# PSeitz/veloci

Measured on AMD Instinct MI355X. Metric: queries/sec, 3-term AND on 100M-doc index (p50 latency and HBM fraction alongside), higher is better.
Workload: dtype u32 doc ids + f16->f32 scores

## Files before the change

veloci_amd/csrc/capi.cpp:

```cpp
#include <chrono>
#include <thread>
#include <cstdio>
#include <cstdlib>
#include <cstring>

#include "../../include/veloci_amd.h"
#include <functional>
#include <future>

#include <dlfcn.h>
#include <unistd.h>

#include "engine.hpp"
#include "text.hpp"

using namespace vq;
using vqreq::Request;
using vqreq::VelociError;

namespace {
thread_local std::string g_err;

int fail(int code, const std::string& msg) {
    g_err = msg;
// ... 1440 lines not shown
        c->nccl = comm;
        comm_setup(idx, std::move(c));
        idx.allreduce_fn = comm_sum_u64;
        idx.allreduce_ctx = &idx;
    });
}
int vq_comm_init_custom(vq_index* index, int nranks, int rank, vq_allgather_fn allgather, vq_allreduce_u32_fn allreduce_u32, void* ctx) {
    return guard([&] {
        if (!index || !allgather || nranks < 1 || rank < 0 || rank >= nranks) throw VelociError(VQ_ERR_INVALID_ARGUMENT, "vq_comm_init_custom: bad argument");
        auto c = std::make_unique<ShardComm>();
        c->nranks = nranks;
        c->rank = rank;
        c->allgather = allgather;
        c->allreduce_u32 = allreduce_u32;
        c->ctx = ctx;
        comm_release(*index->idx, "vq_comm_init_custom");
        comm_setup(*index->idx, std::move(c));
    });
}
int vq_comm_destroy(vq_index* index) {
    return guard([&] {
        if (!index) throw VelociError(VQ_ERR_INVALID_ARGUMENT, "vq_comm_destroy: null index");
        comm_release(*index->idx, "vq_comm_destroy");
    });
}

struct vq_shard_step {
    const Index* idx = nullptr;
    std::vector<std::unique_ptr<PartialBatch>> pbs;
    std::vector<size_t> first, arena_off;
    size_t n = 0, used = 0;
    int parity = 0;
    bool merge_queued = false;
    bool counted = false;
    ~vq_shard_step() {
        pbs.clear();
        if (idx && idx->comm && idx->comm->unmerged == this) idx->comm->unmerged = nullptr;
        if (counted && idx && idx->comm) {
            idx->comm->live -= 1;
            idx->comm->busy[parity] = false;
        }
    }
};
namespace {
void comm_fail(ShardComm& c, const std::string& why) {
    if (!c.failed.empty()) return;
    c.failed = why;
    if (c.nccl) {
        try {
            if (rccl_api().CommAbort) (void)rccl_api().CommAbort(static_cast<ncclComm_t>(c.nccl));
            c.nccl = nullptr;
        } catch (...) {
        }
    }
}
void bounded_wait(const Index& idx, ShardComm& c, hipEvent_t ev) {
    static const long limit_ms = [] {
        const char* e = std::getenv("VQ_STEP_TIMEOUT_MS");
        return e ? std::atol(e) : 120000L;
    }();
    const auto t0 = std::chrono::steady_clock::now();
    for (uint64_t spins = 0;; ++spins) {
        const hipError_t q = hipEventQuery(ev);
        if (q == hipSuccess) return;
        if (q != hipErrorNotReady) {
            comm_fail(c, std::string("the step's stream reported ") + hipGetErrorString(q));
            throw VelociError(VQ_ERR_DEVICE, "sharded step: " + c.failed);
        }
        if (spins < 2000) continue;
        if ((spins & 63u) == 0) {
            if (c.nccl && rccl_api().CommGetAsyncError) {
                int aerr = 0;
                if (rccl_api().CommGetAsyncError(static_cast<ncclComm_t>(c.nccl), &aerr) == 0 && aerr != 0) {
                    comm_fail(c, std::string("RCCL reported ") + (rccl_api().GetErrorString ? rccl_api().GetErrorString(aerr) : "an error") + " while the step was in flight (a rank is gone)");
                    throw VelociError(VQ_ERR_DEVICE, "sharded step: " + c.failed);
                }
            }
            const long waited = long(std::chrono::duration_cast<std::chrono::milliseconds>(std::chrono::steady_clock::now() - t0).count());
            if (limit_ms > 0 && waited > limit_ms) {
                comm_fail(c, "a step did not complete within " + std::to_string(limit_ms) + " ms (VQ_STEP_TIMEOUT_MS): a rank did not join its exchange");
                throw VelociError(VQ_ERR_DEVICE, "sharded step: " + c.failed);
            }
        }
        std::this_thread::sleep_for(std::chrono::microseconds(20));
    }
    (void)idx;
}
void step_queue_merge(vq_shard_step& step) {
    if (step.merge_queued) return;
    step.merge_queued = true;
    const Index& idx = *step.idx;
    ShardComm& c = *idx.comm;
    if (c.unmerged == &step) c.unmerged = nullptr;
    if (step.used) VQ_HIP(hipStreamWaitEvent(idx.fin_stream, c.ev_xchg[step.parity], 0));
    const uint8_t* gathered = static_cast<const uint8_t*>(c.gathered[step.parity].p);
    for (size_t k = 0; k < step.pbs.size(); ++k)
        finish_launch(idx, *step.pbs[k], step.used && step.pbs[k]->nq_dev ? gathered + step.arena_off[k] : nullptr, uint32_t(c.nranks));
    VQ_HIP(hipEventRecord(c.ev_fin[step.parity], idx.fin_stream));
}
}

int vq_shard_step_begin(const vq_index* index, const vq_request* const* requests, size_t n, vq_shard_step** out) {
    return guard([&] {
        if (!index || !out || (n && !requests)) throw VelociError(VQ_ERR_INVALID_ARGUMENT, "vq_shard_step_begin: null argument");
        *out = nullptr;
        const Index& idx = *index->idx;
        if (!idx.comm) {
            auto local = std::make_unique<ShardComm>();
            comm_setup(const_cast<Index&>(idx), std::move(local));
        }
        ShardComm& c = *idx.comm;
        if (!c.failed.empty()) throw VelociError(VQ_ERR_DEVICE, "vq_shard_step_begin: the communicator is down (" + c.failed + "): make it again (vq_comm_init / vq_comm_init_custom) on every rank");
        const bool exchange = c.nccl != nullptr || c.allgather != nullptr;
        static const bool timing = std::getenv("VQ_TIMING") != nullptr;
        const auto tb0 = std::chrono::steady_clock::now();
        VQ_HIP(hipSetDevice(idx.device));
        const std::vector<const Request*> reqs = request_pointers(requests, n);
        if (c.unmerged) {
            vq_shard_step& prev = *static_cast<vq_shard_step*>(c.unmerged);
            step_queue_merge(prev);
            VQ_HIP(hipStreamWaitEvent(idx.stream, c.ev_fin[prev.parity], 0));
        }
        const auto tb1 = std::chrono::steady_clock::now();
        if (c.live >= 2) throw VelociError(VQ_ERR_INVALID_ARGUMENT, "vq_shard_step_begin: two steps are in flight already (end one first)");
        auto step = std::make_unique<vq_shard_step>();
        step->idx = &idx;
        step->counted = true;
        c.live += 1;
        step->n = n;
        step->parity = c.busy[0] ? 1 : 0;
        if (c.busy[step->parity]) {
            step->counted = false;
            c.live -= 1;
            throw VelociError(VQ_ERR_INVALID_ARGUMENT, "vq_shard_step_begin: both step slots are held (end a step first)");
        }
        c.busy[step->parity] = true;
        auto tb2 = tb1;
        try {
        const size_t chunks_env = [] {
            const char* e = std::getenv("VQ_SHARD_CHUNKS");
            return size_t(e ? std::min(2, std::max(1, std::atoi(e))) : 0);
        }();
        const size_t nchunks = chunks_env && n >= 512 ? chunks_env : 1;
        for (size_t k = 0; k < nchunks; ++k) {
            const size_t b = n * k / nchunks, e = n * (k + 1) / nchunks;
            step->first.push_back(b);
            step->pbs.push_back(run_partial(idx, reqs.data() + b, e - b, step->parity * 2 + int(k)));
        }
        tb2 = std::chrono::steady_clock::now();
        size_t off = 0;
        for (auto& pb : step->pbs) {
            step->arena_off.push_back(off);
            if (exchange && pb->nq_dev) off += (size_t(pb->layout.off_hist) * size_t(c.nranks) + 255) / 256 * 256;
        }
// ... 132 lines not shown
```

veloci_amd/csrc/device_types.hpp:

```cpp
#pragma once
#include <hip/hip_runtime.h>
#include <stdint.h>

namespace vq {

constexpr int kBlock = 64;
constexpr int kCandCap = 2048;
constexpr int kMaxTopK = 1024;
constexpr int kStackDepth = 16;
constexpr int kMaxChildren = 16;
constexpr int kMaxLists = 64;
constexpr int kMaxOps = 160;
constexpr int kMaxSkipWhen = 4;
constexpr uint32_t kTileDirShift = 14;
constexpr uint32_t kProbeTileShift = 15;
static_assert(kProbeTileShift == 15, "an arr16 entry holds a 15-bit in-tile offset and a class bit");
constexpr uint32_t kArrPadRel = (1u << kProbeTileShift) - 1u;
#ifndef VQ_SCORE_CLASS_DIV
#define VQ_SCORE_CLASS_DIV 8
#endif
constexpr uint32_t kScoreClassDiv = VQ_SCORE_CLASS_DIV;
constexpr uint32_t kRankShift = 9;

enum ListFlags : uint32_t {
// ... 105 lines not shown
};

constexpr int kWideMax = 16;
struct DWide {
    uint8_t n_leaves, n_groups, root_kind, root_nslots;
    uint8_t seq, pad0, pad1, pad2;
    uint16_t bitmap_mask, cover_mask, prefetch_mask, f32_mask;
    uint16_t leaf_list[kWideMax];
    uint8_t leaf_slot[kWideMax];
    uint8_t g_kind[kWideMax], g_begin[kWideMax], g_count[kWideMax];
    uint8_t leaf_and_order[kWideMax];
    uint8_t leaf_slot_order[kWideMax];
    uint8_t r_and_order[kWideMax];
    uint8_t r_slot[kWideMax];
    uint8_t r_slot_order[kWideMax];
};

struct QHeader {
    uint32_t n_lists, n_ops, n_fops, n_groups, n_tboost, n_col, n_locf, n_facets;
    uint32_t off_lists, off_ops, off_fops, off_groups, off_tboost, off_col, off_locf, off_facets;
    uint32_t top_k;
    uint32_t tile_words;
    uint32_t n_spans;
    uint32_t keys_base;
    uint32_t doc_lo, doc_hi;
    uint32_t part_keys_off;
    uint32_t blob_bytes;
    uint32_t desc_bytes;
    uint32_t n_pres, off_pres, off_pres_in, n_temps;
    uint32_t off_loc_idx;
    uint32_t off_simple2;
    uint32_t off_pool;
    uint32_t prune_n;
    uint64_t prune_mask;
    unsigned long long gthr;
    unsigned long long key_upper;
    uint32_t seq_tiles;
    uint32_t stat_off;
    uint32_t prune_gbits[16];
    uint32_t n_counts;
    uint32_t bitmap_base;
    uint32_t simple_n;
    uint32_t simple_flags;
};

constexpr uint32_t kSfBitmapShift = 0;
constexpr uint32_t kSfCoverShift = 8;
constexpr uint32_t kSfArrayShift = 12;
constexpr uint32_t kSfPrefetchShift = 20;
constexpr uint32_t kSfLeafMask = 0xFu;
constexpr uint32_t kSfSeq = 1u << 16;
constexpr uint32_t kSfSimple = 1u << 17;
constexpr uint32_t kSfRich = 1u << 18;
constexpr uint32_t kSfLeafF32 = 1u << 19;
constexpr uint32_t kSfWide = 1u << 24;
constexpr uint32_t kSfProbe = 1u << 25;
constexpr uint32_t kSfProbeOr = 1u << 27;
constexpr uint32_t kSfUnionPacked = 1u << 28;
__host__ __device__ inline uint32_t sf_bitmap_mask(uint32_t f) { return (f >> kSfBitmapShift) & kSfLeafMask; }
__host__ __device__ inline uint32_t sf_cover_mask(uint32_t f) { return (f >> kSfCoverShift) & kSfLeafMask; }
__host__ __device__ inline uint32_t sf_array_mask(uint32_t f) { return (f >> kSfArrayShift) & kSfLeafMask; }
__host__ __device__ inline uint32_t sf_prefetch_mask(uint32_t f) { return (f >> kSfPrefetchShift) & kSfLeafMask; }
__host__ __device__ inline bool sf_bitmap(uint32_t f, uint32_t k) { return (f >> (kSfBitmapShift + k)) & 1u; }
__host__ __device__ inline bool sf_cover(uint32_t f, uint32_t k) { return (f >> (kSfCoverShift + k)) & 1u; }
__host__ __device__ inline bool sf_array(uint32_t f, uint32_t k) { return (f >> (kSfArrayShift + k)) & 1u; }
__host__ __device__ inline bool sf_prefetch(uint32_t f, uint32_t k) { return (f >> (kSfPrefetchShift + k)) & 1u; }
__host__ __device__ inline bool sf_seq(uint32_t f) { return (f & kSfSeq) != 0u; }
__host__ __device__ inline bool sf_rich(uint32_t f) { return (f & kSfRich) != 0u; }
__host__ __device__ inline bool sf_leaf_f32(uint32_t f) { return (f & kSfLeafF32) != 0u; }
__host__ __device__ inline bool sf_wide(uint32_t f) { return (f & kSfWide) != 0u; }
__host__ __device__ inline bool sf_probe(uint32_t f) { return (f & kSfProbe) != 0u; }
__host__ __device__ inline bool sf_probe_or(uint32_t f) { return (f & kSfProbeOr) != 0u; }
__host__ __device__ inline bool sf_union_packed(uint32_t f) { return (f & kSfUnionPacked) != 0u; }

struct DProbeLeaf {
    const uint32_t* cov32;
    const uint16_t* arr16;
// ... 21 lines not shown
```

veloci_amd/csrc/engine.hpp:

```cpp
#pragma once
#include <hip/hip_runtime.h>

#include <atomic>
#include <cmath>
#include <chrono>
#include <cstdint>
#include <cstdlib>
#include <map>
#include <limits>
#include <memory>
#include <thread>
#include <functional>
#include <condition_variable>
#include <mutex>
#include <string>
#include <unordered_map>
#include <vector>

#include "device_types.hpp"
#include "kernels.hpp"
#include "request.hpp"
#include "hostpool.hpp"
#include "regex_dfa.hpp"

// ... 373 lines not shown
struct PinnedBuf {
    void* p = nullptr;
    size_t bytes = 0;
    PinnedBuf() = default;
    PinnedBuf(const PinnedBuf&) = delete;
    PinnedBuf& operator=(const PinnedBuf&) = delete;
    ~PinnedBuf();
    void ensure(size_t n);
    template <class T>
    T* as() const { return reinterpret_cast<T*>(p); }
};

constexpr int kWorkspaces = 4;

enum KernelId : int {
    K_DICT_SCAN = 0, K_DICT_REGEX, K_DICT_TOPN_GROUP, K_DICT_TOPN, K_TEXT_BEST, K_TEXT_SELECT, K_UNION_COUNT, K_UNION_WRITE, K_UNION_DENSE_SCATTER, K_UNION_DENSE_COUNT, K_UNION_DENSE_WRITE, K_RANGE_HITS, K_COUNT_PREPASS, K_SCAN_LEAF_F32, K_SCAN_RICH, K_SCAN_PROBE, K_SCAN_AND, K_SCAN_SIMPLE, K_SCAN_UNION,
    K_SCAN_WIDE, K_TILE_SCAN, K_MERGE_SPANS, K_FINALIZE, K_FACET_SELECT, K_LOCALITY, K_BOOST1N, K_COUNT_
};
extern const char* const kKernelNames[K_COUNT_];

struct TimedLaunch {
    int kernel;
    uint32_t ev_begin, ev_end;
    uint64_t layout_bytes, algorithmic_bytes, queries;
};

struct Workspace {
    std::mutex mu;
    std::atomic<bool> pinned{false};
    std::vector<hipEvent_t> ev_pool;
    uint32_t ev_used = 0;
    std::vector<TimedLaunch> timed;
    hipEvent_t ev_done = nullptr;
    PinnedBuf h_up, h_down;
    DevBuf d_up;
    DevBuf d_span_keys;
    DevBuf d_partial;
    DevBuf d_down;
    DevBuf d_union_docs[2], d_union_vals[2], d_union_max, d_union_meta;
    DevBuf d_union_slab, d_union_dense_docs, d_union_dense_vals, d_union_dense_meta;
    DevBuf d_loc_a, d_loc_b, d_loc_pairs_a, d_loc_pairs_b, d_loc_meta, d_loc_tmp, d_loc_docs, d_loc_vals;
    DevBuf d_b1n_a, d_b1n_b, d_b1n_meta, d_b1n_tmp, d_b1n_docs, d_b1n_vals;
    DevBuf d_probe_desc, d_probe_counts, d_probe_ids;
    DevBuf d_regex_tabs;
    DevBuf d_topn_sort, d_topn_tmp, d_topn_meta, d_topn_out;
    DevBuf d_trank_best, d_trank_meta;
};

struct KernelProfile {
    double ms = 0;
    uint64_t launches = 0;
    uint64_t layout_bytes = 0;
    uint64_t algorithmic_bytes = 0;
    uint64_t gathered_bytes = 0;
    uint64_t queries = 0;
};
struct Profile {
    bool enabled = false;
    KernelProfile k[K_COUNT_];
    uint64_t batches = 0;
};
struct LaunchTimer {
    Workspace* ws = nullptr;
    hipStream_t st = nullptr;
    size_t slot = 0;
    LaunchTimer(bool on, Workspace& w, hipStream_t s, int kernel, uint64_t layout_bytes = 0, uint64_t algorithmic_bytes = 0, uint64_t queries = 0);
// ... 248 lines not shown
    bool has_facets = false;
    std::map<std::string, std::vector<std::string>> why_found_terms;
    std::shared_ptr<const ExplainPlan> explain_plan;
    std::shared_ptr<const WhyFoundPlan> why_found_plan;
    std::map<uint32_t, std::map<std::string, std::vector<std::string>>> why_found_info;
    bool has_explain = false;
    std::vector<std::pair<bool, ExplainRecs>> explain;
    bool deep = false;
    bool rerun_exact = false;
    mutable std::string json;
};

struct PartialBatch {
    const Index* index = nullptr;
    Workspace* ws = nullptr;
    std::unique_lock<std::mutex> lock;
    bool pinned_ws = false;
    std::vector<CompiledQuery> queries;
    std::vector<uint32_t> slot;
    std::vector<uint8_t> qclass;
    std::vector<FacetJob> facet_jobs;
    uint32_t nq_dev = 0;
    PartialLayout layout{};
    const uint8_t* d_blobs = nullptr;
    const uint32_t* d_blob_off = nullptr;
    const FacetJob* d_facet_jobs = nullptr;
    uint8_t* d_partial = nullptr;
    uint32_t total_spans = 0;
    uint32_t n_facet_jobs = 0;
    uint32_t total_facet_out = 0;
    bool profiled = false;
    bool launched = false, finished = false;
    bool merge_launched = false;
    std::chrono::steady_clock::time_point t0;
    void release_workspace();
    std::vector<const vqreq::Request*> reqs;
    ~PartialBatch();
};

std::unique_ptr<PartialBatch> run_partial(const Index& idx, const vqreq::Request* const* reqs, size_t n, int slot = -1, int64_t arena_offset = -1);
void finish_batch(const Index& idx, PartialBatch& pb, const void* gathered_device, uint32_t num_shards, std::vector<std::unique_ptr<Result>>& out,
                  std::vector<int>& status, std::vector<std::string>& errors, size_t shard_stride = 0);
void finish_launch(const Index& idx, PartialBatch& pb, const void* gathered_device, uint32_t num_shards, size_t shard_stride = 0);

}
```

veloci_amd/csrc/exec.cpp:

```cpp
#include <algorithm>
#include <cstdio>
#include <cstdlib>
#include <cstring>
#include <thread>

#include "engine.hpp"
#include "staging.hpp"

#include "text.hpp"

namespace vq {

using namespace vqreq;

void DevBuf::ensure(size_t n) {
    if (n <= bytes) return;
    size_t want = std::max(n, bytes + bytes / 2);
    alloc(want);
}
PinnedBuf::~PinnedBuf() {
    if (p) (void)hipHostFree(p);
}
void PinnedBuf::ensure(size_t n) {
    if (n <= bytes) return;
// ... 641 lines not shown
                P.facets_rich = P.facets_rich || !cq.facets.empty();
                P.scatter_rich = std::max<uint32_t>(P.scatter_rich, n_scatter + cq.simple2.n_side);
                break;
            case K_SCAN_UNION: P.union_has_or = P.union_has_or || cq.simple_n > 1; break;
            case K_SCAN_PROBE: {
                ScanPlan::ProbeParams& pp = P.probe[ti - T_PROBE];
                pp.na_seen |= 1u << uint32_t(__builtin_popcount(sf_array_mask(cq.simple_flags)));
                pp.arr_slot = std::max(pp.arr_slot, cq.probe_arr_gran * 4u);
                P.any_probe = true;
                break;
            }
            case K_SCAN_AND: P.scatter_and = std::max(P.scatter_and, n_scatter); break;
            case K_SCAN_SIMPLE: P.scatter_simple = std::max(P.scatter_simple, n_scatter); break;
            default: break;
        }
        pb.qclass.push_back(uint8_t(cq.kclass));
        P.cls_layout[cq.kclass] += cq.layout_bytes;
        P.cls_algo[cq.kclass] += cq.algorithmic_bytes;
        P.cls_q[cq.kclass] += 1;
        ++qi;
    }
    for (ScanTable& t : P.tabs) t.span_base[t.n] = t.spans;
    if (!pb.facet_jobs.empty()) std::memcpy(hup + up_jobs, pb.facet_jobs.data(), pb.facet_jobs.size() * sizeof(FacetJob));
    pb.d_blobs = dup;
    pb.d_blob_off = reinterpret_cast<const uint32_t*>(dup + up_blob_off);
    pb.d_facet_jobs = reinterpret_cast<const FacetJob*>(dup + up_jobs);
    return P;
}

static void launch_scans(const Index& idx, PartialBatch& pb, const BatchLayout& L, const ScanPlan& P, int64_t arena_offset) {
    Workspace& ws = *pb.ws;
    const PartialLayout& lay = pb.layout;
    hipStream_t st = idx.stream;
    VQ_HIP(hipMemcpyAsync(ws.d_up.as<uint8_t>(), ws.h_up.as<uint8_t>(), P.up_bytes, hipMemcpyHostToDevice, st));
    ws.d_span_keys.ensure(size_t(L.total_span_keys) * 8 + 16);
    if (arena_offset >= 0) {
        if (size_t(arena_offset) % 256 || size_t(arena_offset) + lay.bytes > Index::kArenaBytes)
            throw VelociError(ERR_UNSUPPORTED, "partial arena: the step's partials do not fit (" + std::to_string(size_t(arena_offset) + lay.bytes) + " bytes)");
        idx.arena.ensure(Index::kArenaBytes);
        pb.d_partial = idx.arena.as<uint8_t>() + arena_offset;
    } else {
        ws.d_partial.ensure(lay.bytes);
        pb.d_partial = ws.d_partial.as<uint8_t>();
    }
    VQ_HIP(hipMemsetAsync(pb.d_partial, 0, lay.bytes, st));

    uint32_t max_top_k = 1;
    uint32_t desc_cap = 0;
    bool facets_generic = false;
    static const bool no_facet_cache = std::getenv("VQ_NO_FACET_CACHE") != nullptr;
    for (const CompiledQuery& cq : pb.queries) {
        if (cq.status != 0) continue;
        max_top_k = std::max(max_top_k, cq.top_k);
        desc_cap = std::max(desc_cap, uint32_t(cq.desc_bytes));
        if (cq.kclass == K_TILE_SCAN && !cq.facets.empty()) facets_generic = !no_facet_cache;
    }
    desc_cap = uint32_t(align_up(desc_cap, 16));
    if (facets_generic) desc_cap += 2 * 1024 * 4;
    static const uint32_t cand_min = [] {
        const char* e = std::getenv("VQ_CAND_CAP");
        return uint32_t(e ? std::max(32, std::atoi(e)) : 32);
    }();
    uint32_t cand_cap = cand_min;
    while (cand_cap < 2 * max_top_k) cand_cap <<= 1;
    const uint32_t list_table = (std::max<uint32_t>(L.max_lists, 2) + 1u) & ~1u;
    static const bool tile_queue = std::getenv("VQ_NO_QUEUE") == nullptr;
    size_t lds_bytes = 0;
    for (const CompiledQuery& cq : pb.queries)
        if (cq.status == 0 && cq.kclass == K_TILE_SCAN)
            lds_bytes = std::max(lds_bytes, tile_scan_lds_bytes(uint32_t(cq.lists.size()) + cq.n_temps, uint32_t(cq.lists.size()), cq.tile_words, L.stack_depth, cand_cap, desc_cap,
                                                                tile_queue && !cq.simple_n, list_table));
    if (lds_bytes > 160 * 1024) throw VelociError(ERR_UNSUPPORTED, "LDS tile larger than 160 KiB");

    auto hits_ptr = reinterpret_cast<unsigned long long*>(pb.d_partial + lay.off_hits);
    auto hist_ptr = reinterpret_cast<uint32_t*>(pb.d_partial + lay.off_hist);
    auto keys_ptr = ws.d_span_keys.as<unsigned long long>();
    auto scan = [&](uint32_t table, int k, auto&& launch) {
        if (const ScanTable& t = P.tabs[table]; t.spans) {
            LaunchTimer lt(pb.profiled, ws, st, k, P.cls_layout[k], P.cls_algo[k], P.cls_q[k]);
            launch(t);
        }
        VQ_HIP(hipGetLastError());
    };
    scan(T_LEAF_F32, K_SCAN_LEAF_F32, [&](const ScanTable& t) { launch_scan_leaf_f32(st, t.spans, pb.d_blobs, pb.d_blob_off, t.d_span_base, t.d_qmap, t.n, cand_cap, keys_ptr, hits_ptr, hist_ptr); });
    scan(T_RICH, K_SCAN_RICH, [&](const ScanTable& t) { launch_scan_simple(st, true, P.scatter_rich, t.spans, pb.d_blobs, pb.d_blob_off, t.d_span_base, t.d_qmap, t.n, cand_cap, keys_ptr, hits_ptr, hist_ptr, P.facets_rich); });
    if (P.any_probe) {
        LaunchTimer lt(pb.profiled, ws, st, K_SCAN_PROBE, P.cls_layout[K_SCAN_PROBE], P.cls_algo[K_SCAN_PROBE], P.cls_q[K_SCAN_PROBE]);
        static const bool trace = std::getenv("VQ_PROBE_TRACE") != nullptr;
        for (uint32_t c = 0; c < kProbeShapes; ++c)
            if (const ScanTable& t = P.tabs[T_PROBE + c]; t.spans && trace)
                std::fprintf(stderr, "probe launch: shape %u, %u queries, %u spans, array slot %u words (fullest tile: %u granules), NA seen 0x%x\n", c, t.n, t.spans,
                             P.probe[c].arr_slot, P.probe[c].arr_slot / 4, P.probe[c].na_seen);
        for (uint32_t c = 0; c < kProbeShapes; ++c)
            if (const ScanTable& t = P.tabs[T_PROBE + c]; t.spans)
                launch_scan_probe_shape(st, c, P.probe[c].na_seen, P.probe[c].arr_slot, t.spans, pb.d_blobs, pb.d_blob_off, t.d_span_base, t.d_qmap, t.n, cand_cap, keys_ptr, hits_ptr);
    }
    VQ_HIP(hipGetLastError());
    scan(T_AND, K_SCAN_AND, [&](const ScanTable& t) { launch_scan_simple(st, false, P.scatter_and, t.spans, pb.d_blobs, pb.d_blob_off, t.d_span_base, t.d_qmap, t.n, cand_cap, keys_ptr, hits_ptr, hist_ptr); });
    scan(T_SIMPLE, K_SCAN_SIMPLE, [&](const ScanTable& t) { launch_scan_simple(st, false, P.scatter_simple, t.spans, pb.d_blobs, pb.d_blob_off, t.d_span_base, t.d_qmap, t.n, cand_cap, keys_ptr, hits_ptr, hist_ptr); });
    scan(T_UNION, K_SCAN_UNION, [&](const ScanTable& t) { launch_scan_union(st, P.union_has_or, t.spans, pb.d_blobs, pb.d_blob_off, t.d_span_base, t.d_qmap, t.n, cand_cap, keys_ptr, hits_ptr); });
    scan(T_WIDE, K_SCAN_WIDE, [&](const ScanTable& t) { launch_scan_wide(st, P.leaves_wide, P.scatter_wide, t.spans, pb.d_blobs, pb.d_blob_off, t.d_span_base, t.d_qmap, t.n, cand_cap, keys_ptr, hits_ptr); });
    scan(T_TILE, K_TILE_SCAN, [&](const ScanTable& t) { launch_tile_scan(st, t.spans, lds_bytes, pb.d_blobs, pb.d_blob_off, t.d_span_base, t.d_qmap, t.n, L.stack_depth, cand_cap, desc_cap, keys_ptr, hits_ptr, hist_ptr, tile_queue, list_table, facets_generic); });
    {
        LaunchTimer t(pb.profiled, ws, st, K_MERGE_SPANS, L.total_span_keys * 8 + L.total_keys * 8, L.total_span_keys * 8 + L.total_keys * 8, L.nq);
        launch_merge_spans(st, L.nq, pb.d_blobs, pb.d_blob_off, keys_ptr, reinterpret_cast<unsigned long long*>(pb.d_partial + lay.off_keys));
    }
    VQ_HIP(hipGetLastError());
    VQ_HIP(hipEventRecord(ws.ev_done, st));
    pb.launched = true;
}

static void report_timing(size_t n, double t_start, const CompileReport& c, double t_layout, double t_packed, const ScanTable* tabs) {
    if (!timing_enabled()) return;
    std::fprintf(stderr, "[vq timing] n=%zu compile %.3f ms (dictionary scans %.3f [%zu probes], pass 1 %.3f, unions %.3f [%zu jobs], pass 2 %.3f), range jobs %.3f [%zu], spans generic/simple/and/rich/union %u/%u/%u/%u/%u, pack+launch %.3f ms\n", n,
                 c.t_compiled - t_start, c.t_probes - t_start, c.probes, c.t_pass1 - c.t_probes, c.t_unions - c.t_pass1, c.unions, c.t_compiled - c.t_ranges,
                 c.t_ranges - c.t_unions, c.ranges, tabs[T_TILE].spans, tabs[T_SIMPLE].spans, tabs[T_AND].spans, tabs[T_RICH].spans, tabs[T_UNION].spans + tabs[T_LEAF_F32].spans, now_ms() - c.t_compiled);
    std::fprintf(stderr, "[vq timing] pack+launch: span sizing + layout %.3f, blobs + tables %.3f, upload + launches %.3f ms\n", t_layout - c.t_compiled, t_packed - t_layout, now_ms() - t_packed);
    uint64_t v[16];
    for (int k = 0; k < 16; ++k) v[k] = g_compile_ns[k].exchange(0);
    if (std::getenv("VQ_TIMING_SUB")) {
        std::fprintf(stderr, "[vq timing] inside 1:n resolve (thread-ms; 6 value-id gather, 7 sort, 8 pairs, 9 order check + layers):");
        for (int k = 6; k < 10; ++k) std::fprintf(stderr, " [%d] %.3f", k, v[k] * 1e-6);
        std::fprintf(stderr, "\n");
    }
    std::fprintf(stderr, "[vq timing] compile thread-ms: total %.3f = dictionary lookups %.3f + 1:n resolve %.3f + 1:n layers %.3f + leaf lists %.3f + rest %.3f; longest request %.3f\n", v[5] * 1e-6,
                 v[0] * 1e-6, v[1] * 1e-6, (v[2] - v[1]) * 1e-6, v[3] * 1e-6, (double(v[5]) - double(v[0]) - double(v[2]) - double(v[3])) * 1e-6, v[4] * 1e-6);
}

std::unique_ptr<PartialBatch> run_partial(const Index& idx, const vqreq::Request* const* reqs, size_t n, int slot, int64_t arena_offset) {
    const double t_start = now_ms();
    auto pb = std::make_unique<PartialBatch>();
    pb->index = &idx;
    pb->reqs.assign(reqs, reqs + n);
    pb->t0 = std::chrono::steady_clock::now();
    acquire_workspace(idx, *pb, slot);
    VQ_HIP(hipSetDevice(idx.device));
// ... 725 lines not shown
struct DownLayout {
    size_t K, J, F, o_hits, o_n, o_ids, o_scores, o_fn, o_fv, o_fc, o_stat, bytes;
    explicit DownLayout(const PartialBatch& pb) {
        const uint32_t nq = pb.nq_dev;
        K = size_t(pb.layout.total_keys);
        J = pb.n_facet_jobs;
        F = pb.total_facet_out;
        o_hits = 0;
        o_n = align_up(o_hits + size_t(nq) * 8, 16);
        o_ids = align_up(o_n + size_t(nq) * 4, 16);
        o_scores = align_up(o_ids + K * 4, 16);
        o_fn = align_up(o_scores + K * 4, 16);
        o_fv = align_up(o_fn + J * 4, 16);
        o_fc = align_up(o_fv + F * 4, 16);
        o_stat = align_up(o_fc + F * 4, 16);
        bytes = align_up(o_stat + size_t(nq) * 8, 256);
    }
};
}

void finish_launch(const Index& idx, PartialBatch& pb, const void* gathered_device, uint32_t num_shards, size_t shard_stride) {
    if (pb.merge_launched) return;
    pb.merge_launched = true;
    Workspace& ws = *pb.ws;
    hipStream_t st = idx.fin_stream;
    const PartialLayout& lay = pb.layout;
    const uint32_t nq = pb.nq_dev;
    VQ_HIP(hipSetDevice(idx.device));
    const DownLayout D(pb);
    const size_t K = D.K, J = D.J;
    if (!nq) return;
    const uint8_t* gathered = gathered_device ? static_cast<const uint8_t*>(gathered_device) : pb.d_partial;
    if (!gathered_device) num_shards = 1;
    ws.d_down.ensure(D.bytes);
    ws.h_down.ensure(D.bytes);
    if (st != idx.stream) VQ_HIP(hipStreamWaitEvent(st, ws.ev_done, 0));
    uint8_t* dd = ws.d_down.as<uint8_t>();
    const bool prof = pb.profiled;
    {
        LaunchTimer t(prof, ws, st, K_FINALIZE, uint64_t(num_shards) * (K * 8 + nq * 8) + K * 8, uint64_t(num_shards) * (K * 8 + nq * 8) + K * 8, nq);
        launch_finalize(st, nq, pb.d_blobs, pb.d_blob_off, gathered, num_shards, shard_stride ? shard_stride : size_t(lay.off_hist), lay, reinterpret_cast<uint32_t*>(dd + D.o_ids),
                        reinterpret_cast<float*>(dd + D.o_scores), reinterpret_cast<uint32_t*>(dd + D.o_n), reinterpret_cast<unsigned long long*>(dd + D.o_hits));
    }
    VQ_HIP(hipGetLastError());
    if (J) {
        const uint32_t* hist = reinterpret_cast<const uint32_t*>(pb.d_partial + lay.off_hist);
        LaunchTimer t(prof, ws, st, K_FACET_SELECT, lay.total_hist * 4, lay.total_hist * 4, J);
        launch_facet_select(st, uint32_t(J), pb.d_facet_jobs, hist, reinterpret_cast<uint32_t*>(dd + D.o_fv), reinterpret_cast<uint32_t*>(dd + D.o_fc),
                            reinterpret_cast<uint32_t*>(dd + D.o_fn));
        VQ_HIP(hipGetLastError());
    }
    VQ_HIP(hipMemcpyAsync(ws.h_down.p, dd, D.o_stat, hipMemcpyDeviceToHost, st));
    if (prof)
        VQ_HIP(hipMemcpyAsync(ws.h_down.as<uint8_t>() + D.o_stat, pb.d_partial + lay.off_stats, size_t(nq) * 8, hipMemcpyDeviceToHost, st));
}

void finish_batch(const Index& idx, PartialBatch& pb, const void* gathered_device, uint32_t num_shards, std::vector<std::unique_ptr<Result>>& out,
                  std::vector<int>& status, std::vector<std::string>& errors, size_t shard_stride) {
    const size_t n = pb.queries.size();
    out.clear();
    out.resize(n);
    status.assign(n, 0);
    errors.assign(n, std::string());
    finish_launch(idx, pb, gathered_device, num_shards, shard_stride);
    Workspace& ws = *pb.ws;
    hipStream_t st = idx.fin_stream;
    const PartialLayout& lay = pb.layout;
    const uint32_t nq = pb.nq_dev;
    const DownLayout D(pb);
    const size_t o_hits = D.o_hits, o_n = D.o_n, o_ids = D.o_ids, o_scores = D.o_scores, o_fn = D.o_fn, o_fv = D.o_fv, o_fc = D.o_fc;
    if (nq) {
        const bool prof = pb.profiled;
        VQ_HIP(hipStreamSynchronize(st));
        const uint64_t* gathered_bytes = reinterpret_cast<const uint64_t*>(ws.h_down.as<uint8_t>() + D.o_stat);
        pb.finished = true;
        if (prof) {
            std::lock_guard<std::mutex> g(idx.profile_mutex);
            Profile& P = idx.profile;
            account_timed_launches(P, ws);
            for (uint32_t q = 0; q < nq && q < pb.qclass.size(); ++q) {
                P.k[pb.qclass[q]].layout_bytes += gathered_bytes[q];
                P.k[pb.qclass[q]].gathered_bytes += gathered_bytes[q];
            }
        }
    }
    const uint64_t ns = uint64_t(std::chrono::duration_cast<std::chrono::nanoseconds>(std::chrono::steady_clock::now() - pb.t0).count());
    const double t_synced = now_ms();

    const uint8_t* hd = ws.h_down.as<uint8_t>();
    size_t key_off = 0, job = 0, fac_off = 0;
    for (size_t i = 0; i < n; ++i) {
        const CompiledQuery& cq = pb.queries[i];
        if (cq.status != 0) {
            status[i] = cq.status;
            errors[i] = cq.error;
            continue;
        }
        const uint32_t q = pb.slot[i];
        auto r = std::make_unique<Result>();
        r->num_hits = reinterpret_cast<const uint64_t*>(hd + o_hits)[q];
        r->execution_time_ns = ns;
        const uint32_t have = reinterpret_cast<const uint32_t*>(hd + o_n)[q];
        const uint32_t* ids = reinterpret_cast<const uint32_t*>(hd + o_ids) + key_off;
        const float* scores = reinterpret_cast<const float*>(hd + o_scores) + key_off;
        const uint32_t want = cq.top + cq.skip;
        const uint32_t avail = std::min(have, want);
// ... 81 lines not shown
```

veloci_amd/csrc/index.cpp:

```cpp
#include <algorithm>
#include <atomic>
#include <chrono>
#include <cstring>
#include <exception>
#include <mutex>
#include <thread>
#include <sys/mman.h>

#include "engine.hpp"
#include "text.hpp"

namespace vq {

uint16_t score_class_pivot(const uint16_t* sc, uint32_t len, uint16_t max_raw) {
    if (len == 0 || max_raw >= 0x7C00u) return max_raw;
    std::vector<uint32_t> count(size_t(max_raw) + 1, 0u);
    for (uint32_t i = 0; i < len; ++i) ++count[sc[i]];
    const uint64_t need = (uint64_t(len) + kScoreClassDiv - 1) / kScoreClassDiv;
    uint64_t above = 0;
    for (uint32_t r = max_raw; r-- > 0;) {
        above += count[r + 1];
        if (above >= need && count[r]) return uint16_t(r);
    }
    return max_raw;
// ... 8 lines not shown
const char* const ANCHOR_TO_TEXT_ID = ".anchor_to_text_id";
const char* const BOOST_VALID_TO_VALUE = ".boost_valid_to_value";
const char* const TOKEN_VALUES = ".token_values";
const char* const VALUE_ID_TO_ANCHOR = ".value_id_to_anchor";
const char* const TEXTINDEX = ".textindex";

static bool ends_with(const std::string& s, const char* suf) {
    size_t n = std::strlen(suf);
    return s.size() >= n && std::memcmp(s.data() + s.size() - n, suf, n) == 0;
}

void DevBuf::alloc(size_t n) {
    release();
    bytes = n;
    if (n == 0) return;
    VQ_HIP(hipMalloc(&p, n));
}
void DevBuf::release() {
    if (p) (void)hipFree(p);
    p = nullptr;
    bytes = 0;
}
void DevBuf::upload(const void* src, size_t n, hipStream_t st) {
    if (n == 0) return;
    if (st) VQ_HIP(hipMemcpyAsync(p, src, n, hipMemcpyHostToDevice, st));
    else VQ_HIP(hipMemcpy(p, src, n, hipMemcpyHostToDevice));
}

Index::~Index() {
    for (auto& w : ws) {
        for (auto e : w.ev_pool)
            if (e) (void)hipEventDestroy(e);
        if (w.ev_done) (void)hipEventDestroy(w.ev_done);
    }
    if (own_stream) (void)hipStreamDestroy(own_stream);
    if (own_fin_stream) (void)hipStreamDestroy(own_fin_stream);
    if (pre_stream) (void)hipStreamDestroy(pre_stream);
}

bool Index::is_anchor_identity(const std::string& textindex_path) const {
    std::string field = textindex_path;
    if (ends_with(field, TEXTINDEX)) field.resize(field.size() - std::strlen(TEXTINDEX));
    auto it = columns.find(field);
    return it != columns.end() && it->second.is_anchor_identity_column;
}

static uint16_t f32_to_f16_rne(float f) {
    uint32_t x;
    std::memcpy(&x, &f, 4);
    const uint32_t sign = (x >> 16) & 0x8000u;
    const uint32_t exp = (x >> 23) & 0xFFu;
    uint32_t man = x & 0x7FFFFFu;
    if (exp == 0xFF) return uint16_t(sign | 0x7C00u | (man ? (0x200u | (man >> 13)) : 0));
    const int32_t e = int32_t(exp) - 112;
    if (e >= 0x1F) return uint16_t(sign | 0x7C00u);
    if (e <= 0) {
        if (e < -10) return uint16_t(sign);
        man |= 0x800000u;
        const uint32_t shift = uint32_t(14 - e);
        uint32_t hm = man >> shift;
        const uint32_t rb = 1u << (shift - 1);
        if ((man & rb) && ((man & (rb - 1)) || (hm & 1))) hm++;
        return uint16_t(sign | hm);
    }
    uint32_t h = sign | (uint32_t(e) << 10) | (man >> 13);
    if ((man & 0x1000u) && ((man & 0xFFFu) || (h & 1))) h++;
// ... 43 lines not shown
    body();
    for (auto& w : workers) w.join();
    if (err) std::rethrow_exception(err);
}

std::unique_ptr<Index> build_index(const IndexBuilder& b, int device) {
    int ndev = 0;
    hipError_t de = hipGetDeviceCount(&ndev);
    if (de != hipSuccess || ndev <= 0)
        throw VelociError(vqreq::ERR_DEVICE, std::string("no HIP device available (hipGetDeviceCount: ") + hipGetErrorString(de) + ", count " +
                                                 std::to_string(ndev) + "): the veloci_amd query path needs an MI355X (no CPU fallback)");
    if (device < 0 || device >= ndev) throw VelociError(vqreq::ERR_INVALID_ARGUMENT, "device index out of range");
    VQ_HIP(hipSetDevice(device));

    auto idx = std::make_unique<Index>();
    idx->device = device;
    static std::atomic<uint64_t> next_uid{1};
    idx->uid = next_uid.fetch_add(1);
    idx->num_anchors = b.num_anchors;
    idx->doc_lo = b.doc_lo;
    idx->doc_hi = b.doc_hi;
    idx->columns = b.columns;
    VQ_HIP(hipStreamCreateWithFlags(&idx->own_stream, hipStreamNonBlocking));
    {
        int lo = 0, hi = 0;
        VQ_HIP(hipDeviceGetStreamPriorityRange(&lo, &hi));
        VQ_HIP(hipStreamCreateWithPriority(&idx->own_fin_stream, hipStreamNonBlocking, hi));
    }
    VQ_HIP(hipStreamCreateWithFlags(&idx->pre_stream, hipStreamNonBlocking));
    idx->stream = idx->own_stream;
    idx->fin_stream = idx->own_fin_stream;
    for (auto& w : idx->ws) {
        VQ_HIP(hipEventCreateWithFlags(&w.ev_done, hipEventDisableTiming));
    }
    const uint32_t lo = b.doc_lo, hi = b.doc_hi;
    idx->bitmap_base = lo & ~65535u;
    idx->bitmap_words = ((uint64_t(hi) - idx->bitmap_base + 65535u) / 65536u) * 2048u + 2048u;

    for (auto& [path, f] : b.fst) {
        Dictionary d;
        d.terms = f.terms;
        d.lower_map.reserve(d.terms.size());
        for (uint32_t i = 0; i < d.terms.size(); ++i) d.lower_map[vqtext::to_lower_utf8(d.terms[i])].push_back(i);
        {
            std::vector<uint32_t> off(d.terms.size() + 1, 0u);
            std::vector<uint32_t> raw, low;
            std::vector<uint64_t> seen(0x110000 / 64, 0ull);
            for (uint32_t i = 0; i < d.terms.size(); ++i) {
                d.max_term_bytes = std::max(d.max_term_bytes, d.terms[i].size());
                for (uint32_t cp : vqtext::decode_utf8(d.terms[i])) {
                    if (cp < 0x110000u) seen[cp >> 6] |= 1ull << (cp & 63u);
                    else d.alphabet.push_back(cp);
                    if (cp > 0xFFFFu) d.char_bytes = 4;
                    if (cp == 0x130u) d.low_exact = false;
                    raw.push_back(cp);
                    low.push_back(vqtext::lower_cp(cp));
                }
                off[i + 1] = uint32_t(raw.size());
            }
            auto image = [&](DevBuf& dst, const std::vector<uint32_t>& cps) {
                if (d.char_bytes == 4) {
                    dst.alloc(cps.size() * 4 + 16);
                    dst.upload(cps.data(), cps.size() * 4);
                } else {
                    const std::vector<uint16_t> narrow(cps.begin(), cps.end());
                    dst.alloc(narrow.size() * 2 + 16);
// ... 427 lines not shown
```

veloci_amd/csrc/scan_probe.hip:

```cpp
#include <hip/hip_runtime.h>
#include <hip/hip_fp16.h>

#include "device_types.hpp"
#include "kernel_common.hpp"
#include "kernels.hpp"
#include "probe_common.hpp"

namespace vq {

#ifdef VQ_STAMP
__device__ unsigned long long g_probe_stamp[16];
#define PS_INIT                                                      \
    unsigned long long _st0 = __builtin_amdgcn_s_memtime();          \
    const unsigned long long _t0 = _st0;                             \
    const unsigned long long _r0 = __builtin_amdgcn_s_memrealtime(); \
    unsigned long long _acc[16] = {0};
#define PS_AT(k)                                                \
    {                                                           \
        unsigned long long _st1 = __builtin_amdgcn_s_memtime(); \
        _acc[k] += _st1 - _st0;                                 \
        _st0 = _st1;                                            \
    }
#define PS_COUNT(k) _acc[k] += 1ull;
#define PS_FLUSH                                                                                             \
// ... 610 lines not shown
                for (uint32_t r = 0; r < kPMaxR; ++r)
                    if (r < rounds) pw[r] = probe_read(cid[r]);
#pragma unroll
                for (uint32_t r = 0; r < kPMaxR; ++r)
                    if (r < rounds) {
                        PS_COUNT(9)
                        probe_eval(cid[r], pw[r], r > 0u);
                    }
            }
            for (uint32_t r = kPMaxR; r < rounds; ++r) {
                const uint32_t v = v0 + r * 64u + lane;
                u32x4 e4 = kSent;
                if (v < v1) e4 = cc4[v];
                PS_COUNT(9)
                const ProbeWords pw = probe_read(e4);
                probe_eval(e4, pw, true);
            }
            PS_AT(2)
            while (un) {
                PS_COUNT(10)
                rank_some(un < 64u ? un : 64u);
            }
            PS_AT(3)
        }
        ++t;
        tile_lo += kPT;
    }
    while (f_stage || rn) flush_service(true);
    __syncthreads();
    cand_prune(cs, top_k);
    {
        const uint32_t cn = *cand_n;
        unsigned long long* out = span_keys + (size_t)keys_base + (size_t)span * top_k;
        for (uint32_t i = lane; i < top_k; i += 64u) out[i] = i < cn ? cand[i] : 0ull;
    }
    if (OR) {
        uint32_t total;
        (void)wave_excl_scan_u32(ucnt, &total);
        hits += (unsigned long long)total;
    }
    if (lane == 0 && hits) atomicAdd(&num_hits[q], hits);
    if (lane == 0 && H->stat_off && lds[4]) atomicAdd(&num_hits[H->stat_off], (unsigned long long)lds[4]);
    PS_AT(6)
    PS_FLUSH
}

__device__ __forceinline__ void probe_item(const uint32_t* __restrict__ span_base, const uint32_t* __restrict__ qmap, uint32_t nq, uint32_t* q, uint32_t* span) {
    uint32_t lo = 0, hi = nq;
    const uint32_t wg = blockIdx.x;
    while (hi - lo > 1) {
        uint32_t mid = (lo + hi) >> 1;
        if (span_base[mid] <= wg) lo = mid;
        else hi = mid;
    }
    *span = blockIdx.x - span_base[lo];
    *q = qmap[lo];
}

#define VQ_PROBE_PARAMS                                                                                                                                       \
    const uint8_t *__restrict__ blobs, const uint32_t *__restrict__ blob_off, const uint32_t *__restrict__ span_base, const uint32_t *__restrict__ qmap, uint32_t nq, \
        uint32_t cand_cap, uint32_t arr_slot, unsigned long long *__restrict__ span_keys, unsigned long long *__restrict__ num_hits
#define VQ_PROBE_ITEM                           \
    uint32_t q, span;                           \
    probe_item(span_base, qmap, nq, &q, &span); \
    const uint8_t* blob = blobs + blob_off[q];
#ifndef VQ_PROBE_WAVES
#define VQ_PROBE_WAVES 4
#endif
#define VQ_PROBE_KERNEL(waves) __global__ __launch_bounds__(64) __attribute__((amdgpu_waves_per_eu(waves, 8))) void

VQ_PROBE_KERNEL(VQ_PROBE_WAVES) k_scan_probe_1(VQ_PROBE_PARAMS) {
    VQ_PROBE_ITEM
    if (sf_array_mask(as_const<QHeader>(blob)->simple_flags) == 0u) probe_body<1, 0>(blob, span, q, cand_cap, arr_slot, span_keys, num_hits);
    else probe_body<1, 1>(blob, span, q, cand_cap, arr_slot, span_keys, num_hits);
}
// ... 59 lines not shown
```

Before: 178,900.

## Merge span top-k in last-arriving probe workgroup and skip finish kernels

Each probe workgroup takes an atomic ticket on its query header after writing its span keys, and the last one to arrive merges all span candidates into the partial top-k. This removes the separate merge_spans launch. When every query qualifies, the finish step skips its device kernels: it copies the raw partial region to the host and decodes ids and scores there, and the next step no longer waits on the finish event. Upload and memset can also move to a pre-stream. Risks include memory-ordering bugs in the ticket protocol, more host-side decode work, and a header field addition that relies on layout padding.

```diff
diff --git a/veloci_amd/csrc/capi.cpp b/veloci_amd/csrc/capi.cpp
--- a/veloci_amd/csrc/capi.cpp
+++ b/veloci_amd/csrc/capi.cpp
@@ -1496,6 +1496,7 @@
     size_t n = 0, used = 0;
     int parity = 0;
     bool merge_queued = false;
+    bool fin_kernels = false;
     bool counted = false;
     ~vq_shard_step() {
         pbs.clear();
@@ -1560,6 +1561,8 @@
     const uint8_t* gathered = static_cast<const uint8_t*>(c.gathered[step.parity].p);
     for (size_t k = 0; k < step.pbs.size(); ++k)
         finish_launch(idx, *step.pbs[k], step.used && step.pbs[k]->nq_dev ? gathered + step.arena_off[k] : nullptr, uint32_t(c.nranks));
+    for (const auto& pb : step.pbs)
+        if (pb->nq_dev && !pb->copied_raw) step.fin_kernels = true;
     VQ_HIP(hipEventRecord(c.ev_fin[step.parity], idx.fin_stream));
 }
 }
@@ -1583,7 +1586,7 @@
         if (c.unmerged) {
             vq_shard_step& prev = *static_cast<vq_shard_step*>(c.unmerged);
             step_queue_merge(prev);
-            VQ_HIP(hipStreamWaitEvent(idx.stream, c.ev_fin[prev.parity], 0));
+            if (prev.fin_kernels) VQ_HIP(hipStreamWaitEvent(idx.stream, c.ev_fin[prev.parity], 0));
         }
         const auto tb1 = std::chrono::steady_clock::now();
         if (c.live >= 2) throw VelociError(VQ_ERR_INVALID_ARGUMENT, "vq_shard_step_begin: two steps are in flight already (end one first)");
diff --git a/veloci_amd/csrc/device_types.hpp b/veloci_amd/csrc/device_types.hpp
--- a/veloci_amd/csrc/device_types.hpp
+++ b/veloci_amd/csrc/device_types.hpp
@@ -161,6 +161,7 @@
     uint32_t off_simple2;
     uint32_t off_pool;
     uint32_t prune_n;
+    uint32_t span_ticket;
     uint64_t prune_mask;
     unsigned long long gthr;
     unsigned long long key_upper;
@@ -171,7 +172,9 @@
     uint32_t bitmap_base;
     uint32_t simple_n;
     uint32_t simple_flags;
-};
+    unsigned long long* part_keys;
+};
+static_assert(sizeof(QHeader) == 256 && offsetof(QHeader, span_ticket) == 132, "the header keeps its 256 bytes (descriptor and LDS sizes follow it); the ticket fills the gap in front of prune_mask");
 
 constexpr uint32_t kSfBitmapShift = 0;
 constexpr uint32_t kSfCoverShift = 8;
diff --git a/veloci_amd/csrc/engine.hpp b/veloci_amd/csrc/engine.hpp
--- a/veloci_amd/csrc/engine.hpp
+++ b/veloci_amd/csrc/engine.hpp
@@ -429,6 +429,7 @@
     uint32_t ev_used = 0;
     std::vector<TimedLaunch> timed;
     hipEvent_t ev_done = nullptr;
+    hipEvent_t ev_up = nullptr;
     PinnedBuf h_up, h_down;
     DevBuf d_up;
     DevBuf d_span_keys;
@@ -743,6 +744,8 @@
     bool profiled = false;
     bool launched = false, finished = false;
     bool merge_launched = false;
+    bool ticket_merged = false;
+    bool copied_raw = false;
     std::chrono::steady_clock::time_point t0;
     void release_workspace();
     std::vector<const vqreq::Request*> reqs;
diff --git a/veloci_amd/csrc/exec.cpp b/veloci_amd/csrc/exec.cpp
--- a/veloci_amd/csrc/exec.cpp
+++ b/veloci_amd/csrc/exec.cpp
@@ -697,7 +697,6 @@
     Workspace& ws = *pb.ws;
     const PartialLayout& lay = pb.layout;
     hipStream_t st = idx.stream;
-    VQ_HIP(hipMemcpyAsync(ws.d_up.as<uint8_t>(), ws.h_up.as<uint8_t>(), P.up_bytes, hipMemcpyHostToDevice, st));
     ws.d_span_keys.ensure(size_t(L.total_span_keys) * 8 + 16);
     if (arena_offset >= 0) {
         if (size_t(arena_offset) % 256 || size_t(arena_offset) + lay.bytes > Index::kArenaBytes)
@@ -708,7 +707,6 @@
         ws.d_partial.ensure(lay.bytes);
         pb.d_partial = ws.d_partial.as<uint8_t>();
     }
-    VQ_HIP(hipMemsetAsync(pb.d_partial, 0, lay.bytes, st));
 
     uint32_t max_top_k = 1;
     uint32_t desc_cap = 0;
@@ -728,6 +726,29 @@
     }();
     uint32_t cand_cap = cand_min;
     while (cand_cap < 2 * max_top_k) cand_cap <<= 1;
+
+    static const bool no_ticket = std::getenv("VQ_NO_SPAN_TICKET") != nullptr;
+    bool ticket = !no_ticket && L.nq != 0;
+    for (const CompiledQuery& cq : pb.queries)
+        if (cq.status == 0 && !(cq.kclass == K_SCAN_PROBE && cq.top_k >= 1 && cq.top_k <= kPoolMaxK && 2 * cq.top_k <= cand_cap)) ticket = false;
+    pb.ticket_merged = ticket;
+    if (ticket) {
+        uint8_t* hup = ws.h_up.as<uint8_t>();
+        const uint32_t* hbo = reinterpret_cast<const uint32_t*>(hup + (reinterpret_cast<const uint8_t*>(pb.d_blob_off) - pb.d_blobs));
+        for (uint32_t q = 0; q < L.nq; ++q) {
+            QHeader* h = reinterpret_cast<QHeader*>(hup + hbo[q]);
+            h->part_keys =reinterpret_cast<unsigned long long*>(pb.d_partial + lay.off_keys);
+        }
+    }
+    {
+        hipStream_t up = (st == idx.own_stream && arena_offset < 0 && idx.pre_stream) ? idx.pre_stream : st;
+        VQ_HIP(hipMemcpyAsync(ws.d_up.as<uint8_t>(), ws.h_up.as<uint8_t>(), P.up_bytes, hipMemcpyHostToDevice, up));
+        VQ_HIP(hipMemsetAsync(pb.d_partial, 0, lay.bytes, up));
+        if (up != st) {
+            VQ_HIP(hipEventRecord(ws.ev_up, up));
+            VQ_HIP(hipStreamWaitEvent(st, ws.ev_up, 0));
+        }
+    }
     const uint32_t list_table = (std::max<uint32_t>(L.max_lists, 2) + 1u) & ~1u;
     static const bool tile_queue = std::getenv("VQ_NO_QUEUE") == nullptr;
     size_t lds_bytes = 0;
@@ -766,7 +787,7 @@
     scan(T_UNION, K_SCAN_UNION, [&](const ScanTable& t) { launch_scan_union(st, P.union_has_or, t.spans, pb.d_blobs, pb.d_blob_off, t.d_span_base, t.d_qmap, t.n, cand_cap, keys_ptr, hits_ptr); });
     scan(T_WIDE, K_SCAN_WIDE, [&](const ScanTable& t) { launch_scan_wide(st, P.leaves_wide, P.scatter_wide, t.spans, pb.d_blobs, pb.d_blob_off, t.d_span_base, t.d_qmap, t.n, cand_cap, keys_ptr, hits_ptr); });
     scan(T_TILE, K_TILE_SCAN, [&](const ScanTable& t) { launch_tile_scan(st, t.spans, lds_bytes, pb.d_blobs, pb.d_blob_off, t.d_span_base, t.d_qmap, t.n, L.stack_depth, cand_cap, desc_cap, keys_ptr, hits_ptr, hist_ptr, tile_queue, list_table, facets_generic); });
-    {
+    if (!pb.ticket_merged) {
         LaunchTimer t(pb.profiled, ws, st, K_MERGE_SPANS, L.total_span_keys * 8 + L.total_keys * 8, L.total_span_keys * 8 + L.total_keys * 8, L.nq);
         launch_merge_spans(st, L.nq, pb.d_blobs, pb.d_blob_off, keys_ptr, reinterpret_cast<unsigned long long*>(pb.d_partial + lay.off_keys));
     }
@@ -1558,9 +1579,14 @@
     if (!nq) return;
     const uint8_t* gathered = gathered_device ? static_cast<const uint8_t*>(gathered_device) : pb.d_partial;
     if (!gathered_device) num_shards = 1;
+    pb.copied_raw = pb.ticket_merged && !gathered_device && !J;
     ws.d_down.ensure(D.bytes);
-    ws.h_down.ensure(D.bytes);
+    ws.h_down.ensure(D.bytes + (pb.copied_raw ? size_t(lay.off_hist) : 0));
     if (st != idx.stream) VQ_HIP(hipStreamWaitEvent(st, ws.ev_done, 0));
+    if (pb.copied_raw) {
+        VQ_HIP(hipMemcpyAsync(ws.h_down.as<uint8_t>() + D.bytes, pb.d_partial + lay.off_hits, size_t(lay.off_hist - lay.off_hits), hipMemcpyDeviceToHost, st));
+        return;
+    }
     uint8_t* dd = ws.d_down.as<uint8_t>();
     const bool prof = pb.profiled;
     {
@@ -1598,6 +1624,29 @@
     if (nq) {
         const bool prof = pb.profiled;
         VQ_HIP(hipStreamSynchronize(st));
+        if (pb.copied_raw) {
+            uint8_t* down = ws.h_down.as<uint8_t>();
+            const uint8_t* raw = down + D.bytes;
+            std::memcpy(down + o_hits, raw, size_t(nq) * 8);
+            std::memcpy(down + D.o_stat, raw + (lay.off_stats - lay.off_hits), size_t(nq) * 8);
+            const uint64_t* keys = reinterpret_cast<const uint64_t*>(raw + (lay.off_keys - lay.off_hits));
+            uint32_t* ids = reinterpret_cast<uint32_t*>(down + o_ids);
+            uint32_t* score_bits = reinterpret_cast<uint32_t*>(down + o_scores);
+            uint32_t* have = reinterpret_cast<uint32_t*>(down + o_n);
+            size_t at = 0;
+            for (const CompiledQuery& cq : pb.queries) {
+                if (cq.status != 0) continue;
+                uint32_t n_keys = 0;
+                for (uint32_t i = 0; i < cq.top_k; ++i) {
+                    const uint64_t k = keys[at + i];
+                    ids[at + i] = uint32_t(k & 0xFFFFFFFFull);
+                    score_bits[at + i] = unorder_f32(uint32_t(k >> 32));
+                    n_keys += k != 0 ? 1u : 0u;
+                }
+                *have++ = n_keys;
+                at += cq.top_k;
+            }
+        }
         const uint64_t* gathered_bytes = reinterpret_cast<const uint64_t*>(ws.h_down.as<uint8_t>() + D.o_stat);
         pb.finished = true;
         if (prof) {
diff --git a/veloci_amd/csrc/index.cpp b/veloci_amd/csrc/index.cpp
--- a/veloci_amd/csrc/index.cpp
+++ b/veloci_amd/csrc/index.cpp
@@ -64,6 +64,7 @@
         for (auto e : w.ev_pool)
             if (e) (void)hipEventDestroy(e);
         if (w.ev_done) (void)hipEventDestroy(w.ev_done);
+        if (w.ev_up) (void)hipEventDestroy(w.ev_up);
     }
     if (own_stream) (void)hipStreamDestroy(own_stream);
     if (own_fin_stream) (void)hipStreamDestroy(own_fin_stream);
@@ -173,6 +174,7 @@
     idx->fin_stream = idx->own_fin_stream;
     for (auto& w : idx->ws) {
         VQ_HIP(hipEventCreateWithFlags(&w.ev_done, hipEventDisableTiming));
+        VQ_HIP(hipEventCreateWithFlags(&w.ev_up, hipEventDisableTiming));
     }
     const uint32_t lo = b.doc_lo, hi = b.doc_hi;
     idx->bitmap_base = lo & ~65535u;
diff --git a/veloci_amd/csrc/scan_probe.hip b/veloci_amd/csrc/scan_probe.hip
--- a/veloci_amd/csrc/scan_probe.hip
+++ b/veloci_amd/csrc/scan_probe.hip
@@ -666,7 +666,11 @@
     {
         const uint32_t cn = *cand_n;
         unsigned long long* out = span_keys + (size_t)keys_base + (size_t)span * top_k;
-        for (uint32_t i = lane; i < top_k; i += 64u) out[i] = i < cn ? cand[i] : 0ull;
+        if (H->part_keys) {
+            for (uint32_t i = lane; i < top_k; i += 64u) __hip_atomic_store(out + i, i < cn ? cand[i] : 0ull, __ATOMIC_RELAXED, __HIP_MEMORY_SCOPE_AGENT);
+        } else {
+            for (uint32_t i = lane; i < top_k; i += 64u) out[i] = i < cn ? cand[i] : 0ull;
+        }
     }
     if (OR) {
         uint32_t total;
@@ -675,6 +679,37 @@
     }
     if (lane == 0 && hits) atomicAdd(&num_hits[q], hits);
     if (lane == 0 && H->stat_off && lds[4]) atomicAdd(&num_hits[H->stat_off], (unsigned long long)lds[4]);
+    if (H->part_keys) {
+        __builtin_amdgcn_fence(__ATOMIC_RELEASE, "workgroup");
+        __builtin_amdgcn_s_waitcnt(0x0F70);
+        uint32_t ticket = 0u;
+        if (lane == 0)
+            ticket = __hip_atomic_fetch_add(reinterpret_cast<uint32_t*>(const_cast<uint8_t*>(blob) + offsetof(QHeader, span_ticket)), 1u, __ATOMIC_RELAXED, __HIP_MEMORY_SCOPE_AGENT);
+        ticket = (uint32_t)__builtin_amdgcn_readfirstlane((int)ticket);
+        if (ticket + 1u == n_spans) {
+            __builtin_amdgcn_fence(__ATOMIC_ACQUIRE, "workgroup");
+            const CandState ms{cand, cand_n, thr, cand_cap};
+            const unsigned long long* src = span_keys + (size_t)keys_base;
+            if (lane == 0) {
+                *thr = 0ull;
+                *cand_n = 0;
+            }
+            __syncthreads();
+            const uint32_t per_round = (cand_cap - top_k) / top_k;
+            for (uint32_t s0 = 0; s0 < n_spans; s0 += per_round) {
+                const uint32_t cnt = (n_spans - s0 < per_round ? n_spans - s0 : per_round) * top_k;
+                const uint32_t base = *cand_n;
+                __syncthreads();
+                for (uint32_t i = lane; i < cnt; i += 64u) cand[base + i] = __hip_atomic_load(src + (size_t)s0 * top_k + i, __ATOMIC_RELAXED, __HIP_MEMORY_SCOPE_AGENT);
+                __syncthreads();
+                if (lane == 0) *cand_n = base + cnt;
+                cand_prune(ms, top_k, true);
+            }
+            unsigned long long* part = H->part_keys + H->part_keys_off;
+            const uint32_t mn = *cand_n;
+            for (uint32_t i = lane; i < top_k; i += 64u) part[i] = i < mn ? cand[i] : 0ull;
+        }
+    }
     PS_AT(6)
     PS_FLUSH
 }
```

After: 180,300, median of 6. About the same (+0.8%).
